# brown-ivl/manus

Measured on AMD Instinct MI355X. Metric: train iters/sec (fwd+bwd) 300k Gaussians @1080p, 8 views; PSNR parity, higher is better.
Workload: dtype f32

## Files before the change

### manus_amd/csrc/image_loss.hip

```cpp
#include "mgr_common.h"
#include "il_list.h"
#include <cstdlib>

#define IL_ACC_SLOTS 64
#define IL_NX (IL_ND + 2 * IL_H1)

struct IlWindow {
    float g[11];
};

typedef mgr_v2f v2f;
__device__ __forceinline__ v2f il_v2(float a) { v2f r = {a, a}; return r; }

__global__ __launch_bounds__(IL_T) void k_image_loss(int H, int W, const float* __restrict__ pred,
                                                     const float* __restrict__ target, IlWindow win, float w_l1,
                                                     float w_ssim, float grad_scale, float* __restrict__ dL_dpred,
                                                     float2* __restrict__ partial, const uint32_t* __restrict__ work_list,
                                                     const uint32_t* __restrict__ work_count, int gxb, int gyb,
                                                     unsigned long long* __restrict__ acc_slots, uint32_t nb, float sum_lim,
                                                     uint32_t* __restrict__ bad_flag) {
    __shared__ v2f s_mix[5][3][IL_NX];
    __shared__ float s_red[4];
    const int tid = threadIdx.x;
    const uint32_t n_work = min(*work_count, nb);
    long long acc_l1 = 0, acc_ss = 0;
    unsigned long long acc_px = 0;
    bool bad = false;
  for (uint32_t wi = blockIdx.x; wi < n_work; wi += gridDim.x) {
    const uint32_t bid = work_list[wi];
    const int bxi = (int)(bid % (uint32_t)gxb), byi = (int)((bid / (uint32_t)gxb) % (uint32_t)gyb), v = (int)(bid / (uint32_t)(gxb * gyb));
    const int w0 = bxi * IL_W, h0 = byi * 2;
    const bool row1 = h0 + 1 < H;
    __syncthreads();
    const size_t plane = (size_t)H * W;
    const float* px = pred + (size_t)v * 3 * plane + (size_t)h0 * W;
    const float* py = target + (size_t)v * 3 * plane + (size_t)h0 * W;
    const v2f m0 = il_v2(win.g[5]), m1 = il_v2(win.g[4]), m2 = il_v2(win.g[3]);

    for (int t = tid; t < IL_NX; t += IL_T) {
        const int w = w0 - 2 * IL_H1 + t;
        v2f x[3], y[3];
#pragma unroll
        for (int c = 0; c < 3; ++c) x[c] = y[c] = il_v2(0.f);
        if (w >= 0 && w < W) {
#pragma unroll
            for (int c = 0; c < 3; ++c) {
                x[c].x = px[c * plane + w];
                y[c].x = py[c * plane + w];
                if (row1) {
                    x[c].y = px[c * plane + W + w];
                    y[c].y = py[c * plane + W + w];
                }
            }
        }
        const v2f q[5][3] = {{x[0], x[1], x[2]},
                             {y[0], y[1], y[2]},
                             {x[0] * x[0], x[1] * x[1], x[2] * x[2]},
                             {y[0] * y[0], y[1] * y[1], y[2] * y[2]},
                             {x[0] * y[0], x[1] * y[1], x[2] * y[2]}};
#pragma unroll
        for (int s5 = 0; s5 < 5; ++s5) {
            s_mix[s5][0][t] = m0 * q[s5][0] + m1 * q[s5][1] + m2 * q[s5][2];
            s_mix[s5][1][t] = m1 * q[s5][0] + m0 * q[s5][1] + m1 * q[s5][2];
            s_mix[s5][2][t] = m2 * q[s5][0] + m1 * q[s5][1] + m0 * q[s5][2];
        }
    }
    __syncthreads();

    const float C1 = 0.01f * 0.01f, C2 = 0.03f * 0.03f;
    const int u0 = 2 * tid;
    v2f ssim_acc = il_v2(0.f);
    v2f d[2][3][3];
#pragma unroll
    for (int c = 0; c < 3; ++c) {
        v2f e[2][5];
#pragma unroll
        for (int s5 = 0; s5 < 5; ++s5) {
            v2f win12[12];
#pragma unroll
            for (int k = 0; k < 12; ++k) win12[k] = s_mix[s5][c][u0 + k];
            v2f a = il_v2(0.f), b = il_v2(0.f);
#pragma unroll
            for (int i = 0; i < 11; ++i) {
                const v2f gi = il_v2(win.g[i]);
                a += gi * win12[i];
                b += gi * win12[i + 1];
            }
            e[0][s5] = a;
            e[1][s5] = b;
        }
#pragma unroll
        for (int pp = 0; pp < 2; ++pp) {
            const int w = w0 - IL_H1 + u0 + pp;
            const v2f mu1 = e[pp][0], mu2 = e[pp][1];
            const v2f s11 = e[pp][2] - mu1 * mu1, s22 = e[pp][3] - mu2 * mu2, s12 = e[pp][4] - mu1 * mu2;
            const v2f A = 2.f * mu1 * mu2 + C1, B = 2.f * s12 + C2;
            const v2f Cc = mu1 * mu1 + mu2 * mu2 + C1, Dd = s11 + s22 + C2;
            v2f iC, iD;
            iC.x = __builtin_amdgcn_rcpf(Cc.x); iC.y = __builtin_amdgcn_rcpf(Cc.y);
            iD.x = __builtin_amdgcn_rcpf(Dd.x); iD.y = __builtin_amdgcn_rcpf(Dd.y);
            const v2f inv = iC * iD;
            const v2f S = A * B * inv;
            const bool okw = w >= 0 && w < W;
            v2f keep = {okw ? 1.f : 0.f, (okw && row1) ? 1.f : 0.f};
            const bool own = u0 + pp >= IL_H1 && u0 + pp < IL_H1 + IL_W;
            if (own) ssim_acc += S * keep;
            d[pp][0][c] = keep * (2.f * mu2 * (B - A) * inv - S * 2.f * mu1 * iC + S * 2.f * mu1 * iD);
            d[pp][1][c] = keep * (-S * iD);
            d[pp][2][c] = keep * (2.f * A * inv);
        }
    }
    __syncthreads();
#pragma unroll
    for (int pp = 0; pp < 2; ++pp) {
#pragma unroll
        for (int k = 0; k < 3; ++k) {
            const v2f a = d[pp][k][0], b = d[pp][k][1], c = d[pp][k][2];
            s_mix[k][0][u0 + pp] = m0 * a + m1 * b + m2 * c;
            s_mix[k][1][u0 + pp] = m1 * a + m0 * b + m1 * c;
            s_mix[k][2][u0 + pp] = m2 * a + m1 * b + m0 * c;
        }
    }
    __syncthreads();

    v2f l1_acc = il_v2(0.f);
    const int o0 = 2 * tid;
    if (o0 < IL_W) {
#pragma unroll
        for (int c = 0; c < 3; ++c) {
            v2f f[2][3];
#pragma unroll
            for (int k = 0; k < 3; ++k) {
                v2f win12[12];
#pragma unroll
                for (int j = 0; j < 12; ++j) win12[j] = s_mix[k][c][o0 + j];
                v2f a = il_v2(0.f), b = il_v2(0.f);
#pragma unroll
                for (int i = 0; i < 11; ++i) {
                    const v2f gi = il_v2(win.g[i]);
                    a += gi * win12[i];
                    b += gi * win12[i + 1];
                }
                f[0][k] = a;
                f[1][k] = b;
            }
#pragma unroll
            for (int pp = 0; pp < 2; ++pp) {
                const int w = w0 + o0 + pp;
                if (o0 + pp < IL_W && w < W) {
                    v2f x, y;
                    x.x = px[c * plane + w];
                    y.x = py[c * plane + w];
                    x.y = row1 ? px[c * plane + W + w] : 0.f;
                    y.y = row1 ? py[c * plane + W + w] : 0.f;
                    const v2f dS = f[pp][0] + 2.f * x * f[pp][1] + y * f[pp][2];
                    const v2f df = x - y;
                    v2f ad = {fabsf(df.x), fabsf(df.y)};
                    l1_acc += ad;
                    const v2f sgn = {df.x > 0.f ? 1.f : (df.x < 0.f ? -1.f : 0.f), df.y > 0.f ? 1.f : (df.y < 0.f ? -1.f : 0.f)};
                    const v2f gr = grad_scale * (w_l1 * sgn - w_ssim * dS);
                    float* go = dL_dpred + (size_t)v * 3 * plane + (size_t)h0 * W + c * plane + w;
                    go[0] = gr.x;
                    if (row1) go[W] = gr.y;
                }
            }
        }
    }
    float l1_sum = mgr_wave_sum63(l1_acc.x + l1_acc.y);
    float ssim_sum = mgr_wave_sum63(ssim_acc.x + ssim_acc.y);
    if ((tid & 63) == 63) {
        s_red[tid >> 6] = l1_sum;
        s_red[2 + (tid >> 6)] = ssim_sum;
    }
    __syncthreads();
    if (tid == 0) {
        const float pa = s_red[0] + s_red[1], pb = s_red[2] + s_red[3];
        partial[bid] = make_float2(pa, pb);
        bad |= !(fabsf(pa) <= sum_lim && fabsf(pb) <= sum_lim);
        acc_l1 += __double2ll_rn((double)pa * 4294967296.0);
        acc_ss += __double2ll_rn((double)pb * 4294967296.0);
        acc_px += (unsigned long long)((min((bxi + 1) * IL_W, W) - bxi * IL_W) * 3 * (row1 ? 2 : 1));
    }
  }
    if (tid == 0 && acc_px) {
        unsigned long long* sl = acc_slots + 3 * (blockIdx.x & (IL_ACC_SLOTS - 1));
        atomicAdd(sl, (unsigned long long)acc_l1);
        atomicAdd(sl + 1, (unsigned long long)acc_ss);
        atomicAdd(sl + 2, acc_px);
        if (bad) atomicOr(bad_flag, 1u);
    }
}

__global__ __launch_bounds__(ILS_T) void k_image_loss_scan(int H, int W, int gxb, const float* __restrict__ pred,
                                                           const float* __restrict__ target, float* __restrict__ dL_dpred,
                                                           float2* __restrict__ partial, uint32_t* __restrict__ work_list,
                                                           uint32_t* __restrict__ work_count) {
    __shared__ uint32_t s_diff[ILS_MAXW / 32];
    __shared__ uint32_t s_ident[(ILS_MAXW / IL_W + 32) / 32];
    const int tid = threadIdx.x;
    const int h0 = blockIdx.x * 2, v = blockIdx.y;
    const bool row1 = h0 + 1 < H;
    const size_t plane = (size_t)H * W;
    const float* px = pred + (size_t)v * 3 * plane + (size_t)h0 * W;
    const float* py = target + (size_t)v * 3 * plane + (size_t)h0 * W;
    float* pg = dL_dpred + (size_t)v * 3 * plane + (size_t)h0 * W;
    const int nwords = (W + 31) / 32;
    for (int k = tid; k < nwords; k += ILS_T) s_diff[k] = 0;
    if (tid < (int)(sizeof(s_ident) / 4)) s_ident[tid] = 0;
    __syncthreads();
    const int rows = row1 ? 2 : 1;
    const bool vec = (W & 3) == 0 && ((((uintptr_t)pred) | ((uintptr_t)target) | ((uintptr_t)dL_dpred)) & 15) == 0;
    if (vec) {
        const int n4 = W >> 2;
        for (int q = tid; q < n4; q += ILS_T) {
            uint32_t d = 0;
#pragma unroll
            for (int c = 0; c < 3; ++c)
                for (int r = 0; r < rows; ++r) {
                    const float4 a = *(const float4*)(px + c * plane + (size_t)r * W + 4 * q);
                    const float4 b = *(const float4*)(py + c * plane + (size_t)r * W + 4 * q);
                    d |= (a.x != b.x ? 1u : 0u) | (a.y != b.y ? 2u : 0u) | (a.z != b.z ? 4u : 0u) | (a.w != b.w ? 8u : 0u);
                }
            if (d) atomicOr(&s_diff[q >> 3], d << ((q & 7) * 4));
        }
    } else {
        for (int w = tid; w < W; w += ILS_T) {
            uint32_t d = 0;
#pragma unroll
            for (int c = 0; c < 3; ++c)
                for (int r = 0; r < rows; ++r) d |= px[c * plane + (size_t)r * W + w] != py[c * plane + (size_t)r * W + w] ? 1u : 0u;
            if (d) atomicOr(&s_diff[w >> 5], 1u << (w & 31));
        }
    }
    __syncthreads();
    for (int b = tid; b < gxb; b += ILS_T) {
        const int lo = max(b * IL_W - 2 * IL_H1, 0), hi = min(b * IL_W + IL_ND, W);
        uint32_t any = 0;
        for (int k = lo >> 5; k <= (hi - 1) >> 5; ++k) {
            uint32_t m = s_diff[k];
            const int base = k << 5;
            if (lo > base) m &= ~0u << (lo - base);
            if (hi < base + 32) m &= ~0u >> (base + 32 - hi);
            any |= m;
        }
        const uint32_t bid = ((uint32_t)v * gridDim.x + blockIdx.x) * (uint32_t)gxb + (uint32_t)b;
        if (any) {
            work_list[atomicAdd(work_count, 1u)] = bid;
        } else {
            atomicOr(&s_ident[b >> 5], 1u << (b & 31));
            const int wcnt = min((b + 1) * IL_W, W) - b * IL_W;
            partial[bid] = make_float2(0.f, (float)(wcnt * 3 * rows));
        }
    }
    __syncthreads();
    if (vec) {
        const int n4 = W >> 2;
        for (int q = tid; q < n4; q += ILS_T) {
            const int w = 4 * q, b0 = w / IL_W, b1 = (w + 3) / IL_W;
            const bool i0 = (s_ident[b0 >> 5] >> (b0 & 31)) & 1u, i1 = (s_ident[b1 >> 5] >> (b1 & 31)) & 1u;
            if (i0 && i1) {
#pragma unroll
                for (int c = 0; c < 3; ++c)
                    for (int r = 0; r < rows; ++r) *(float4*)(pg + c * plane + (size_t)r * W + w) = make_float4(0.f, 0.f, 0.f, 0.f);
            } else if (i0 || i1) {
                for (int e = 0; e < 4; ++e) {
                    const int be = (w + e) / IL_W;
                    if ((s_ident[be >> 5] >> (be & 31)) & 1u)
                        for (int c = 0; c < 3; ++c)
                            for (int r = 0; r < rows; ++r) pg[c * plane + (size_t)r * W + w + e] = 0.f;
                }
            }
        }
    } else {
        for (int w = tid; w < W; w += ILS_T) {
            const int b = w / IL_W;
            if ((s_ident[b >> 5] >> (b & 31)) & 1u)
                for (int c = 0; c < 3; ++c)
                    for (int r = 0; r < rows; ++r) pg[c * plane + (size_t)r * W + w] = 0.f;
        }
    }
}

__global__ __launch_bounds__(ILS_T) void k_image_loss_list(int H, int W, int gxb, const float* __restrict__ target,
                                                           const float* __restrict__ bg, const uint32_t* __restrict__ tile_start,
                                                           float2* __restrict__ partial, uint32_t* __restrict__ work_list,
                                                           uint32_t* __restrict__ work_count, const uint32_t* __restrict__ tmap,
                                                           uint32_t* __restrict__ tmap_out) {
    __shared__ uint32_t s_diff[ILS_MAXW / 32];
    __shared__ uint32_t s_cand[(ILS_MAXW / IL_W + 32) / 32];
    __shared__ uint32_t s_n, s_base;
    const int tid = threadIdx.x;
    if (tid == 0) s_n = 0;
    const int h0 = blockIdx.x * 2, v = blockIdx.y;
    const bool row1 = h0 + 1 < H;
    const size_t plane = (size_t)H * W;
    const float* py = target + (size_t)v * 3 * plane + (size_t)h0 * W;
    const int nwords = (W + 31) / 32;
    const int gxt = (W + 15) / 16, T = gxt * ((H + 15) / 16);
    const uint32_t* trow = tile_start + (size_t)v * T + (size_t)(h0 >> 4) * gxt;
    const size_t map_row = ((size_t)v * gridDim.x + blockIdx.x) * (size_t)nwords;
    for (int k = tid; k < nwords; k += ILS_T) s_diff[k] = tmap ? tmap[map_row + k] : 0u;
    if (tid < (int)(sizeof(s_cand) / 4)) s_cand[tid] = 0;
    __syncthreads();
    if (tile_start)
    for (int b = tid; b < gxb; b += ILS_T) {
        const int lo = max(b * IL_W - 2 * IL_H1, 0), hi = min(b * IL_W + IL_ND, W);
        const int t0 = lo >> 4, t1 = (hi - 1) >> 4;
        if (trow[t1 + 1] == trow[t0]) atomicOr(&s_cand[b >> 5], 1u << (b & 31));
    }
    const int rows = row1 ? 2 : 1;
    const float b0 = bg[0], b1 = bg[1], b2 = bg[2];
    const bool vec = (W & 3) == 0 && (((uintptr_t)target) & 15) == 0;
    if (tmap) {
    } else if (vec) {
        const int n4 = W >> 2;
        for (int q = tid; q < n4; q += ILS_T) {
            uint32_t d = 0;
            for (int rr = 0; rr < rows; ++rr) {
                const float4 c0 = *(const float4*)(py + (size_t)rr * W + 4 * q), c1 = *(const float4*)(py + plane + (size_t)rr * W + 4 * q),
                             c2 = *(const float4*)(py + 2 * plane + (size_t)rr * W + 4 * q);
                d |= ((c0.x != b0 || c1.x != b1 || c2.x != b2) ? 1u : 0u) | ((c0.y != b0 || c1.y != b1 || c2.y != b2) ? 2u : 0u) |
                     ((c0.z != b0 || c1.z != b1 || c2.z != b2) ? 4u : 0u) | ((c0.w != b0 || c1.w != b1 || c2.w != b2) ? 8u : 0u);
            }
            if (d) atomicOr(&s_diff[q >> 3], d << ((q & 7) * 4));
        }
    } else {
        for (int w = tid; w < W; w += ILS_T) {
            uint32_t d = 0;
            for (int rr = 0; rr < rows; ++rr)
                d |= (py[(size_t)rr * W + w] != b0 || py[plane + (size_t)rr * W + w] != b1 || py[2 * plane + (size_t)rr * W + w] != b2) ? 1u : 0u;
            if (d) atomicOr(&s_diff[w >> 5], 1u << (w & 31));
        }
    }
    __syncthreads();
    if (tmap_out) {
        for (int k = tid; k < nwords; k += ILS_T) tmap_out[map_row + k] = s_diff[k];
        if (!tile_start) return;
    }
    uint32_t my_rank[(ILS_MAXW / IL_W + ILS_T) / ILS_T];
    int nmine = 0;
    for (int b = tid; b < gxb; b += ILS_T, ++nmine) {
        const int lo = max(b * IL_W - 2 * IL_H1, 0), hi = min(b * IL_W + IL_ND, W);
        uint32_t any = ((s_cand[b >> 5] >> (b & 31)) & 1u) ? 0u : 1u;
        for (int k = lo >> 5; k <= (hi - 1) >> 5 && !any; ++k) {
            uint32_t m = s_diff[k];
            const int base = k << 5;
            if (lo > base) m &= ~0u << (lo - base);
            if (hi < base + 32) m &= ~0u >> (base + 32 - hi);
            any |= m;
        }
        my_rank[nmine] = any ? atomicAdd(&s_n, 1u) : 0xFFFFFFFFu;
        if (!any) {
            const uint32_t bid = ((uint32_t)v * gridDim.x + blockIdx.x) * (uint32_t)gxb + (uint32_t)b;
            const int wcnt = min((b + 1) * IL_W, W) - b * IL_W;
            partial[bid] = make_float2(0.f, (float)(wcnt * 3 * rows));
        }
    }
    __syncthreads();
    if (tid == 0 && s_n) s_base = atomicAdd(work_count, s_n);
    __syncthreads();
    nmine = 0;
    for (int b = tid; b < gxb; b += ILS_T, ++nmine)
        if (my_rank[nmine] != 0xFFFFFFFFu)
            work_list[s_base + my_rank[nmine]] = ((uint32_t)v * gridDim.x + blockIdx.x) * (uint32_t)gxb + (uint32_t)b;
}

__global__ __launch_bounds__(ILS_T) void k_image_loss_list_mapped(IlListArgs a) {
    __shared__ uint32_t s2[2];
    il_list_mapped_block(a, (int)blockIdx.x, (int)blockIdx.y, s2);
}

__global__ __launch_bounds__(IL_ACC_SLOTS) void k_image_loss_fold(unsigned long long* __restrict__ acc_slots, long long total_px3,
                                                                  float* __restrict__ sums, float ca, float cb, float cc,
                                                                  uint32_t* __restrict__ work_count) {
    __shared__ unsigned long long s_fin[3 * IL_ACC_SLOTS];
    const int tid = threadIdx.x;
#pragma unroll
    for (int q = 0; q < 3; ++q) {
        s_fin[q * IL_ACC_SLOTS + tid] = acc_slots[3 * tid + q];
        acc_slots[3 * tid + q] = 0ull;
    }
    __syncthreads();
    if (tid == 0) {
        long long t_l1 = 0, t_ss = 0;
        unsigned long long t_px = 0;
        for (int k = 0; k < IL_ACC_SLOTS; ++k) {
            t_l1 += (long long)s_fin[k];
            t_ss += (long long)s_fin[IL_ACC_SLOTS + k];
            t_px += s_fin[2 * IL_ACC_SLOTS + k];
        }
        const double ta = (double)t_l1 * (1.0 / 4294967296.0);
        const double tb = (double)t_ss * (1.0 / 4294967296.0) + (double)((unsigned long long)total_px3 - t_px);
        const bool bad = work_count[1] != 0u;
        const float qnan = __int_as_float(0x7FC00000);
        sums[0] = bad ? qnan : (float)ta;
        sums[1] = bad ? qnan : (float)tb;
        sums[2] = bad ? qnan : (float)((double)ca * ta + (double)cb * tb + (double)cc);
        work_count[0] = 0u;
        work_count[1] = 0u;
    }
}


static size_t il_slots_offset(int64_t nb) { return (((size_t)nb * (sizeof(float2) + sizeof(uint32_t)) + 256) + 63) & ~(size_t)63; }
extern "C" size_t mgr_image_loss_workspace_bytes(int V, int H, int W) {
    if (V <= 0 || H <= 0 || W <= 0) return 0;
    return il_slots_offset(il_blocks(V, H, W)) + 3 * IL_ACC_SLOTS * sizeof(unsigned long long);
}

static int image_loss_impl(int V, int H, int W, const float* pred, const float* target, const float* bg3,
                           const uint32_t* tile_start, float w_l1, float w_ssim, float grad_scale, float loss_offset,
                           float* dL_dpred, float* sums, void* workspace, size_t workspace_bytes, void* stream_, int phase = 0,
                           const uint32_t* tmap = nullptr, bool clean = false) {
    if (V <= 0 || H <= 0 || W <= 0) return mgr_fail(MGR_EINVAL, "mgr_image_loss: bad sizes");
    if ((!target && !(phase == 1 && tmap)) || !workspace || (phase != 1 && (!pred || !dL_dpred || !sums))) return mgr_fail(MGR_EINVAL, "mgr_image_loss: null pointer");
    if (H > 65535 || V > 65535) return mgr_fail(MGR_EINVAL, "mgr_image_loss: H and V must fit a grid dimension");
    if (workspace_bytes < mgr_image_loss_workspace_bytes(V, H, W))
        return mgr_fail(MGR_ENOMEM, "mgr_image_loss: workspace too small");
    hipStream_t stream = (hipStream_t)stream_;
    IlWindow win;
    float sum = 0.f;
    for (int i = 0; i < 11; ++i) {
        win.g[i] = (float)exp(-(double)((i - 5) * (i - 5)) / (2.0 * 1.5 * 1.5));
        sum += win.g[i];
    }
    for (int i = 0; i < 11; ++i) win.g[i] /= sum;
    const dim3 grid((W + IL_W - 1) / IL_W, (H + 1) / 2, V);
    const int64_t nb = il_blocks(V, H, W);
    if (nb >= (1ll << 32)) return mgr_fail(MGR_EINVAL, "mgr_image_loss: image batch too large");
    float2* partial = (float2*)workspace;
    uint32_t* work_list = (uint32_t*)((char*)workspace + (size_t)nb * sizeof(float2));
    uint32_t* work_count = (uint32_t*)((char*)workspace + (size_t)nb * (sizeof(float2) + sizeof(uint32_t)) + 64);
    if (W > ILS_MAXW) return mgr_fail(MGR_EINVAL, "mgr_image_loss: image wider than 16384");
    unsigned long long* acc_slots = (unsigned long long*)((char*)workspace + il_slots_offset(nb));
    if (phase != 2 && !clean)
        MGR_HIP(hipMemsetAsync(work_count, 0, (size_t)((char*)(acc_slots + 3 * IL_ACC_SLOTS) - (char*)work_count), stream));
    if (phase == 2) {
    } else if (tile_start && tmap) {
        MGR_PROF("k_image_loss_list", stream);
        const IlListArgs la = il_list_args(V, H, W, tmap, tile_start, workspace);
        hipLaunchKernelGGL(k_image_loss_list_mapped, dim3((unsigned)la.nbx, V), dim3(ILS_T), 0, stream, la);
    } else if (tile_start) {
        MGR_PROF("k_image_loss_list", stream);
        hipLaunchKernelGGL(k_image_loss_list, dim3(grid.y, V), dim3(ILS_T), 0, stream, H, W, (int)grid.x, target, bg3, tile_start,
                           partial, work_list, work_count, tmap, (uint32_t*)nullptr);
    } else {
        MGR_PROF("k_image_loss_scan", stream);
        hipLaunchKernelGGL(k_image_loss_scan, dim3(grid.y, V), dim3(ILS_T), 0, stream, H, W, (int)grid.x, pred, target, dL_dpred,
                           partial, work_list, work_count);
    }
    if (phase == 1) return MGR_OK;
    {
        MGR_PROF("k_image_loss", stream);
#ifndef IL_GRID
#define IL_GRID (256 * 5)
#endif
        const int64_t pb = nb < IL_GRID ? nb : IL_GRID;
        const float sum_lim = (float)(2147483648.0 * (1.0 - 1.0 / 1048576.0) / (double)nb);
        hipLaunchKernelGGL(k_image_loss, dim3((unsigned)pb), dim3(IL_T), 0, stream, H, W, pred, target, win, w_l1, w_ssim,
                           grad_scale, dL_dpred, partial, (const uint32_t*)work_list, (const uint32_t*)work_count,
                           (int)grid.x, (int)grid.y, acc_slots, (uint32_t)nb, sum_lim, work_count + 1);
    }
    hipLaunchKernelGGL(k_image_loss_fold, dim3(1), dim3(IL_ACC_SLOTS), 0, stream, acc_slots, (long long)V * H * W * 3,
                       sums, grad_scale * w_l1, -grad_scale * w_ssim, loss_offset, work_count);
    MGR_LAUNCH_CHECK("k_image_loss", stream, 0);
    return MGR_OK;
}

extern "C" int mgr_image_loss(int V, int H, int W, const float* pred, const float* target, float w_l1, float w_ssim,
                              float grad_scale, float loss_offset, float* dL_dpred, float* sums, void* workspace,
                              size_t workspace_bytes, void* stream_) {
    return image_loss_impl(V, H, W, pred, target, nullptr, nullptr, w_l1, w_ssim, grad_scale, loss_offset, dL_dpred, sums,
                           workspace, workspace_bytes, stream_);
}

extern "C" int mgr_image_loss_tiles(int V, int H, int W, const float* pred, const float* target, const float* bg3,
                                    const uint32_t* tile_start, float w_l1, float w_ssim, float grad_scale, float loss_offset,
                                    float* dL_dpred, float* sums, void* workspace, size_t workspace_bytes, void* stream_) {
    if (!bg3 || !tile_start) return mgr_fail(MGR_EINVAL, "mgr_image_loss_tiles: null pointer");
    return image_loss_impl(V, H, W, pred, target, bg3, tile_start, w_l1, w_ssim, grad_scale, loss_offset, dL_dpred, sums,
                           workspace, workspace_bytes, stream_);
}

extern "C" int mgr_image_loss_tiles_list(int V, int H, int W, const float* target, const float* bg3, const uint32_t* tile_start,
                                         void* workspace, size_t workspace_bytes, void* stream_) {
    if (!bg3 || !tile_start) return mgr_fail(MGR_EINVAL, "mgr_image_loss_tiles_list: null pointer");
    return image_loss_impl(V, H, W, nullptr, target, bg3, tile_start, 0.f, 0.f, 0.f, 0.f, nullptr, nullptr, workspace,
                           workspace_bytes, stream_, 1);
}

extern "C" int mgr_image_loss_tiles_finish(int V, int H, int W, const float* pred, const float* target, float w_l1, float w_ssim,
                                           float grad_scale, float loss_offset, float* dL_dpred, float* sums, void* workspace,
                                           size_t workspace_bytes, void* stream_) {
    return image_loss_impl(V, H, W, pred, target, nullptr, nullptr, w_l1, w_ssim, grad_scale, loss_offset, dL_dpred, sums,
                           workspace, workspace_bytes, stream_, 2);
}

extern "C" size_t mgr_image_loss_target_map_words(int V, int H, int W) {
    if (V <= 0 || H <= 0 || W <= 0) return 0;
    return (size_t)V * ((H + 1) / 2) * ((W + 31) / 32);
}

extern "C" int mgr_image_loss_target_map(int V, int H, int W, const float* target, const float* bg3, uint32_t* map, void* stream_) {
    if (V <= 0 || H <= 0 || W <= 0) return mgr_fail(MGR_EINVAL, "mgr_image_loss_target_map: bad sizes");
    if (!target || !bg3 || !map) return mgr_fail(MGR_EINVAL, "mgr_image_loss_target_map: null pointer");
    if (H > 65535 || V > 65535 || W > ILS_MAXW) return mgr_fail(MGR_EINVAL, "mgr_image_loss_target_map: image too large");
    hipLaunchKernelGGL(k_image_loss_list, dim3((H + 1) / 2, V), dim3(ILS_T), 0, (hipStream_t)stream_, H, W, (W + IL_W - 1) / IL_W,
                       target, bg3, (const uint32_t*)nullptr, (float2*)nullptr, (uint32_t*)nullptr, (uint32_t*)nullptr,
                       (const uint32_t*)nullptr, map);
    MGR_LAUNCH_CHECK("k_image_loss_list", (hipStream_t)stream_, 0);
    return MGR_OK;
}

extern "C" int mgr_image_loss_tiles_list_mapped(int V, int H, int W, const uint32_t* map, const float* bg3, const uint32_t* tile_start,
                                                void* workspace, size_t workspace_bytes, int workspace_kept, void* stream_) {
    if (!map || !bg3 || !tile_start) return mgr_fail(MGR_EINVAL, "mgr_image_loss_tiles_list_mapped: null pointer");
    return image_loss_impl(V, H, W, nullptr, nullptr, bg3, tile_start, 0.f, 0.f, 0.f, 0.f, nullptr, nullptr, workspace,
                           workspace_bytes, stream_, 1, map, workspace_kept != 0);
}
```

Baseline: 775.0.

## Restructure SSIM loss kernel with register-held tiles and software-prefetched next work item

Rewrites the fused L1+SSIM loss kernel so each thread keeps its own pixel pair in registers, prefetches the next work item's pixels while the current one is still being processed, and recomputes the per-channel vertical mix into a smaller shared buffer instead of one large 5x3 shared array. Pixels reused in the gradient stage come from registers rather than being reloaded from global memory. Loads and gradient stores are vectorised as float2 when alignment allows. It also pins waves-per-EU and raises the grid size. The extra barriers per channel and the higher register pressure could offset the gains.

Result: no change. 775.3 (median of 2 runs) (+0.0%).

```diff
diff --git a/manus_amd/csrc/image_loss.hip b/manus_amd/csrc/image_loss.hip
--- a/manus_amd/csrc/image_loss.hip
+++ b/manus_amd/csrc/image_loss.hip
@@ -12,73 +12,157 @@
 typedef mgr_v2f v2f;
 __device__ __forceinline__ v2f il_v2(float a) { v2f r = {a, a}; return r; }
 
-__global__ __launch_bounds__(IL_T) void k_image_loss(int H, int W, const float* __restrict__ pred,
-                                                     const float* __restrict__ target, IlWindow win, float w_l1,
-                                                     float w_ssim, float grad_scale, float* __restrict__ dL_dpred,
-                                                     float2* __restrict__ partial, const uint32_t* __restrict__ work_list,
-                                                     const uint32_t* __restrict__ work_count, int gxb, int gyb,
-                                                     unsigned long long* __restrict__ acc_slots, uint32_t nb, float sum_lim,
-                                                     uint32_t* __restrict__ bad_flag) {
-    __shared__ v2f s_mix[5][3][IL_NX];
+typedef float il_v4f __attribute__((ext_vector_type(4)));
+
+struct IlSpan {
+    int bxi, w0, h0, v;
+    bool row1;
+    size_t base;
+};
+__device__ __forceinline__ IlSpan il_span(uint32_t bid, int gxb, int gyb, int H, int W, size_t plane) {
+    IlSpan s;
+    s.bxi = (int)(bid % (uint32_t)gxb);
+    const int byi = (int)((bid / (uint32_t)gxb) % (uint32_t)gyb);
+    s.v = (int)(bid / (uint32_t)(gxb * gyb));
+    s.w0 = s.bxi * IL_W;
+    s.h0 = byi * 2;
+    s.row1 = s.h0 + 1 < H;
+    s.base = (size_t)s.v * 3 * plane + (size_t)s.h0 * W;
+    return s;
+}
+
+__device__ __forceinline__ void il_load_pair(const float* __restrict__ px, const float* __restrict__ py, size_t plane, int W, int w,
+                                             bool row1, bool vec2, v2f (&x)[2][3], v2f (&y)[2][3]) {
+    const bool in0 = w >= 0 && w < W, in1 = w + 1 >= 0 && w + 1 < W;
+    const int r1 = row1 ? W : 0;
+    if (vec2) {
+        const uint32_t wc = in0 ? (uint32_t)w : 0u;
+#pragma unroll
+        for (int c = 0; c < 3; ++c) {
+            const float* pxc = px + c * plane;
+            const float* pyc = py + c * plane;
+            const float2 a0 = *(const float2*)(pxc + wc), a1 = *(const float2*)(pxc + r1 + wc);
+            const float2 b0 = *(const float2*)(pyc + wc), b1 = *(const float2*)(pyc + r1 + wc);
+            x[0][c].x = in0 ? a0.x : 0.f; x[0][c].y = (in0 && row1) ? a1.x : 0.f;
+            x[1][c].x = in0 ? a0.y : 0.f; x[1][c].y = (in0 && row1) ? a1.y : 0.f;
+            y[0][c].x = in0 ? b0.x : 0.f; y[0][c].y = (in0 && row1) ? b1.x : 0.f;
+            y[1][c].x = in0 ? b0.y : 0.f; y[1][c].y = (in0 && row1) ? b1.y : 0.f;
+        }
+    } else {
+        const uint32_t wc0 = in0 ? (uint32_t)w : 0u, wc1 = in1 ? (uint32_t)(w + 1) : 0u;
+#pragma unroll
+        for (int c = 0; c < 3; ++c) {
+            const float* pxc = px + c * plane;
+            const float* pyc = py + c * plane;
+            const float a00 = pxc[wc0], a01 = (pxc + r1)[wc0], a10 = pxc[wc1], a11 = (pxc + r1)[wc1];
+            const float b00 = pyc[wc0], b01 = (pyc + r1)[wc0], b10 = pyc[wc1], b11 = (pyc + r1)[wc1];
+            x[0][c].x = in0 ? a00 : 0.f; x[0][c].y = (in0 && row1) ? a01 : 0.f;
+            x[1][c].x = in1 ? a10 : 0.f; x[1][c].y = (in1 && row1) ? a11 : 0.f;
+            y[0][c].x = in0 ? b00 : 0.f; y[0][c].y = (in0 && row1) ? b01 : 0.f;
+            y[1][c].x = in1 ? b10 : 0.f; y[1][c].y = (in1 && row1) ? b11 : 0.f;
+        }
+    }
+}
+
+__device__ __forceinline__ void il_mix5(const v2f (&x)[3], const v2f (&y)[3], int c, v2f m0, v2f m1, v2f m2, v2f (&o)[5]) {
+    const v2f q[5][3] = {{x[0], x[1], x[2]},
+                         {y[0], y[1], y[2]},
+                         {x[0] * x[0], x[1] * x[1], x[2] * x[2]},
+                         {y[0] * y[0], y[1] * y[1], y[2] * y[2]},
+                         {x[0] * y[0], x[1] * y[1], x[2] * y[2]}};
+#pragma unroll
+    for (int s5 = 0; s5 < 5; ++s5) {
+        if (c == 0) o[s5] = m0 * q[s5][0] + m1 * q[s5][1] + m2 * q[s5][2];
+        else if (c == 1) o[s5] = m1 * q[s5][0] + m0 * q[s5][1] + m1 * q[s5][2];
+        else o[s5] = m2 * q[s5][0] + m1 * q[s5][1] + m0 * q[s5][2];
+    }
+}
+
+__global__ __launch_bounds__(IL_T) __attribute__((amdgpu_waves_per_eu(4, 4))) void k_image_loss(
+    int H, int W, const float* __restrict__ pred, const float* __restrict__ target, IlWindow win, float w_l1, float w_ssim,
+    float grad_scale, float* __restrict__ dL_dpred, float2* __restrict__ partial, const uint32_t* __restrict__ work_list,
+    const uint32_t* __restrict__ work_count, int gxb, int gyb, unsigned long long* __restrict__ acc_slots, uint32_t nb, float sum_lim,
+    uint32_t* __restrict__ bad_flag) {
+    __shared__ __attribute__((aligned(16))) v2f s_rows[9][IL_NX];
+    __shared__ __attribute__((aligned(16))) v2f s_left[6][2 * IL_H1];
     __shared__ float s_red[4];
     const int tid = threadIdx.x;
     const uint32_t n_work = min(*work_count, nb);
+    if (blockIdx.x >= n_work) return;
     long long acc_l1 = 0, acc_ss = 0;
     unsigned long long acc_px = 0;
     bool bad = false;
-  for (uint32_t wi = blockIdx.x; wi < n_work; wi += gridDim.x) {
+    const size_t plane = (size_t)H * W;
+    const bool vec2 = (W & 1) == 0 && ((((uintptr_t)pred) | ((uintptr_t)target)) & 7) == 0;
+    const bool vec2s = (W & 1) == 0 && (((uintptr_t)dL_dpred) & 7) == 0;
+    const v2f m0 = il_v2(win.g[5]), m1 = il_v2(win.g[4]), m2 = il_v2(win.g[3]);
+    const float C1 = 0.01f * 0.01f, C2 = 0.03f * 0.03f;
+    const int u0 = 2 * tid, o0 = 2 * tid;
+    const int te = 2 * min(tid, IL_H1 - 1);
+
+    uint32_t wi = blockIdx.x;
+    IlSpan sp = il_span(work_list[wi], gxb, gyb, H, W, plane);
+    v2f x[2][3], y[2][3];
+    v2f xe[2][3], ye[2][3];
+    il_load_pair(pred + sp.base, target + sp.base, plane, W, sp.w0 + 2 * tid, sp.row1, vec2, x, y);
+    il_load_pair(pred + sp.base, target + sp.base, plane, W, sp.w0 - 2 * IL_H1 + te, sp.row1, vec2, xe, ye);
+  for (;;) {
     const uint32_t bid = work_list[wi];
-    const int bxi = (int)(bid % (uint32_t)gxb), byi = (int)((bid / (uint32_t)gxb) % (uint32_t)gyb), v = (int)(bid / (uint32_t)(gxb * gyb));
-    const int w0 = bxi * IL_W, h0 = byi * 2;
-    const bool row1 = h0 + 1 < H;
-    __syncthreads();
-    const size_t plane = (size_t)H * W;
-    const float* px = pred + (size_t)v * 3 * plane + (size_t)h0 * W;
-    const float* py = target + (size_t)v * 3 * plane + (size_t)h0 * W;
-    const v2f m0 = il_v2(win.g[5]), m1 = il_v2(win.g[4]), m2 = il_v2(win.g[3]);
-
-    for (int t = tid; t < IL_NX; t += IL_T) {
-        const int w = w0 - 2 * IL_H1 + t;
-        v2f x[3], y[3];
-#pragma unroll
-        for (int c = 0; c < 3; ++c) x[c] = y[c] = il_v2(0.f);
-        if (w >= 0 && w < W) {
-#pragma unroll
-            for (int c = 0; c < 3; ++c) {
-                x[c].x = px[c * plane + w];
-                y[c].x = py[c * plane + w];
-                if (row1) {
-                    x[c].y = px[c * plane + W + w];
-                    y[c].y = py[c * plane + W + w];
-                }
-            }
-        }
-        const v2f q[5][3] = {{x[0], x[1], x[2]},
-                             {y[0], y[1], y[2]},
-                             {x[0] * x[0], x[1] * x[1], x[2] * x[2]},
-                             {y[0] * y[0], y[1] * y[1], y[2] * y[2]},
-                             {x[0] * y[0], x[1] * y[1], x[2] * y[2]}};
-#pragma unroll
-        for (int s5 = 0; s5 < 5; ++s5) {
-            s_mix[s5][0][t] = m0 * q[s5][0] + m1 * q[s5][1] + m2 * q[s5][2];
-            s_mix[s5][1][t] = m1 * q[s5][0] + m0 * q[s5][1] + m1 * q[s5][2];
-            s_mix[s5][2][t] = m2 * q[s5][0] + m1 * q[s5][1] + m0 * q[s5][2];
-        }
-    }
-    __syncthreads();
-
-    const float C1 = 0.01f * 0.01f, C2 = 0.03f * 0.03f;
-    const int u0 = 2 * tid;
+    const uint32_t wn = wi + gridDim.x;
+    const bool more = wn < n_work;
+    const IlSpan ns = il_span(work_list[more ? wn : wi], gxb, gyb, H, W, plane);
+    const int w0 = sp.w0;
+    const bool row1 = sp.row1;
+    if (tid < IL_H1) {
+#pragma unroll
+        for (int cc = 0; cc < 3; ++cc) {
+            const il_v4f px2 = {xe[0][cc].x, xe[0][cc].y, xe[1][cc].x, xe[1][cc].y}, py2 = {ye[0][cc].x, ye[0][cc].y, ye[1][cc].x, ye[1][cc].y};
+            *(il_v4f*)&s_left[cc][2 * tid] = px2;
+            *(il_v4f*)&s_left[3 + cc][2 * tid] = py2;
+        }
+    }
+
     v2f ssim_acc = il_v2(0.f);
     v2f d[2][3][3];
 #pragma unroll
     for (int c = 0; c < 3; ++c) {
+        {
+#pragma unroll
+            for (int pp = 0; pp < 2; ++pp)
+#pragma unroll
+                for (int cc = 0; cc < 3; ++cc) asm("" : "+v"(x[pp][cc]), "+v"(y[pp][cc]));
+            v2f ma[5], mb[5];
+            il_mix5(x[0], y[0], c, m0, m1, m2, ma);
+            il_mix5(x[1], y[1], c, m0, m1, m2, mb);
+#pragma unroll
+            for (int s5 = 0; s5 < 5; ++s5) {
+                const il_v4f pr = {ma[s5].x, ma[s5].y, mb[s5].x, mb[s5].y};
+                *(il_v4f*)&s_rows[s5][2 * IL_H1 + 2 * tid] = pr;
+            }
+            if (tid < IL_H1) {
+                v2f lx[2][3], ly[2][3];
+#pragma unroll
+                for (int cc = 0; cc < 3; ++cc) {
+                    const il_v4f px2 = *(const il_v4f*)&s_left[cc][2 * tid], py2 = *(const il_v4f*)&s_left[3 + cc][2 * tid];
+                    lx[0][cc] = {px2.x, px2.y}; lx[1][cc] = {px2.z, px2.w};
+                    ly[0][cc] = {py2.x, py2.y}; ly[1][cc] = {py2.z, py2.w};
+                }
+                il_mix5(lx[0], ly[0], c, m0, m1, m2, ma);
+                il_mix5(lx[1], ly[1], c, m0, m1, m2, mb);
+#pragma unroll
+                for (int s5 = 0; s5 < 5; ++s5) {
+                    const il_v4f pr = {ma[s5].x, ma[s5].y, mb[s5].x, mb[s5].y};
+                    *(il_v4f*)&s_rows[s5][2 * tid] = pr;
+                }
+            }
+        }
+        __syncthreads();
         v2f e[2][5];
 #pragma unroll
         for (int s5 = 0; s5 < 5; ++s5) {
             v2f win12[12];
 #pragma unroll
-            for (int k = 0; k < 12; ++k) win12[k] = s_mix[s5][c][u0 + k];
+            for (int k = 0; k < 12; ++k) win12[k] = s_rows[s5][u0 + k];
             v2f a = il_v2(0.f), b = il_v2(0.f);
 #pragma unroll
             for (int i = 0; i < 11; ++i) {
@@ -86,6 +170,7 @@
                 a += gi * win12[i];
                 b += gi * win12[i + 1];
             }
+            asm volatile("" : "+v"(a), "+v"(b) : : "memory");
             e[0][s5] = a;
             e[1][s5] = b;
         }
@@ -109,23 +194,52 @@
             d[pp][1][c] = keep * (-S * iD);
             d[pp][2][c] = keep * (2.f * A * inv);
         }
-    }
-    __syncthreads();
-#pragma unroll
-    for (int pp = 0; pp < 2; ++pp) {
-#pragma unroll
-        for (int k = 0; k < 3; ++k) {
+        asm volatile("" : "+v"(ssim_acc));
+        if (c == 0) {
+#pragma unroll
+            for (int k = 0; k < 3; ++k) {
+                const il_v4f pk = {d[0][k][0].x, d[0][k][0].y, d[1][k][0].x, d[1][k][0].y};
+                *(il_v4f*)&s_rows[5 + k][u0] = pk;
+            }
+        } else if (c == 1) {
+            const il_v4f pk = {d[0][0][1].x, d[0][0][1].y, d[1][0][1].x, d[1][0][1].y};
+            *(il_v4f*)&s_rows[8][u0] = pk;
+        }
+        __syncthreads();
+    }
+#pragma unroll
+    for (int k = 0; k < 3; ++k) {
+        const il_v4f pk = *(const il_v4f*)&s_rows[5 + k][u0];
+        d[0][k][0] = {pk.x, pk.y}; d[1][k][0] = {pk.z, pk.w};
+    }
+    {
+        const il_v4f pk = *(const il_v4f*)&s_rows[8][u0];
+        d[0][0][1] = {pk.x, pk.y}; d[1][0][1] = {pk.z, pk.w};
+    }
+#pragma unroll
+    for (int k = 0; k < 3; ++k) {
+        v2f r[2][3];
+#pragma unroll
+        for (int pp = 0; pp < 2; ++pp) {
             const v2f a = d[pp][k][0], b = d[pp][k][1], c = d[pp][k][2];
-            s_mix[k][0][u0 + pp] = m0 * a + m1 * b + m2 * c;
-            s_mix[k][1][u0 + pp] = m1 * a + m0 * b + m1 * c;
-            s_mix[k][2][u0 + pp] = m2 * a + m1 * b + m0 * c;
-        }
-    }
+            r[pp][0] = m0 * a + m1 * b + m2 * c;
+            r[pp][1] = m1 * a + m0 * b + m1 * c;
+            r[pp][2] = m2 * a + m1 * b + m0 * c;
+        }
+#pragma unroll
+        for (int c = 0; c < 3; ++c) {
+            const il_v4f pr = {r[0][c].x, r[0][c].y, r[1][c].x, r[1][c].y};
+            *(il_v4f*)&s_rows[3 * k + c][u0] = pr;
+        }
+    }
+    v2f nx[2][3], ny[2][3], nxe[2][3], nye[2][3];
+    il_load_pair(pred + ns.base, target + ns.base, plane, W, ns.w0 + 2 * tid, ns.row1, vec2, nx, ny);
+    il_load_pair(pred + ns.base, target + ns.base, plane, W, ns.w0 - 2 * IL_H1 + te, ns.row1, vec2, nxe, nye);
     __syncthreads();
 
     v2f l1_acc = il_v2(0.f);
-    const int o0 = 2 * tid;
     if (o0 < IL_W) {
+        float* gbase = dL_dpred + sp.base;
 #pragma unroll
         for (int c = 0; c < 3; ++c) {
             v2f f[2][3];
@@ -133,7 +247,7 @@
             for (int k = 0; k < 3; ++k) {
                 v2f win12[12];
 #pragma unroll
-                for (int j = 0; j < 12; ++j) win12[j] = s_mix[k][c][o0 + j];
+                for (int j = 0; j < 12; ++j) win12[j] = s_rows[3 * k + c][o0 + j];
                 v2f a = il_v2(0.f), b = il_v2(0.f);
 #pragma unroll
                 for (int i = 0; i < 11; ++i) {
@@ -141,28 +255,35 @@
                     a += gi * win12[i];
                     b += gi * win12[i + 1];
                 }
+                asm volatile("" : "+v"(a), "+v"(b) : : "memory");
                 f[0][k] = a;
                 f[1][k] = b;
             }
+            v2f gr2[2];
 #pragma unroll
             for (int pp = 0; pp < 2; ++pp) {
                 const int w = w0 + o0 + pp;
+                gr2[pp] = il_v2(0.f);
                 if (o0 + pp < IL_W && w < W) {
-                    v2f x, y;
-                    x.x = px[c * plane + w];
-                    y.x = py[c * plane + w];
-                    x.y = row1 ? px[c * plane + W + w] : 0.f;
-                    y.y = row1 ? py[c * plane + W + w] : 0.f;
-                    const v2f dS = f[pp][0] + 2.f * x * f[pp][1] + y * f[pp][2];
-                    const v2f df = x - y;
+                    const v2f xo = x[pp][c], yo = y[pp][c];
+                    const v2f dS = f[pp][0] + 2.f * xo * f[pp][1] + yo * f[pp][2];
+                    const v2f df = xo - yo;
                     v2f ad = {fabsf(df.x), fabsf(df.y)};
                     l1_acc += ad;
                     const v2f sgn = {df.x > 0.f ? 1.f : (df.x < 0.f ? -1.f : 0.f), df.y > 0.f ? 1.f : (df.y < 0.f ? -1.f : 0.f)};
                     const v2f gr = grad_scale * (w_l1 * sgn - w_ssim * dS);
-                    float* go = dL_dpred + (size_t)v * 3 * plane + (size_t)h0 * W + c * plane + w;
-                    go[0] = gr.x;
-                    if (row1) go[W] = gr.y;
+                    gr2[pp] = gr;
+                    if (!vec2s) {
+                        float* go = gbase + c * plane + w;
+                        go[0] = gr.x;
+                        if (row1) go[W] = gr.y;
+                    }
                 }
+            }
+            if (vec2s && w0 + o0 < W) {
+                float* go = gbase + c * plane + w0 + o0;
+                *(float2*)go = make_float2(gr2[0].x, gr2[1].x);
+                if (row1) *(float2*)(go + W) = make_float2(gr2[0].y, gr2[1].y);
             }
         }
     }
@@ -179,8 +300,18 @@
         bad |= !(fabsf(pa) <= sum_lim && fabsf(pb) <= sum_lim);
         acc_l1 += __double2ll_rn((double)pa * 4294967296.0);
         acc_ss += __double2ll_rn((double)pb * 4294967296.0);
-        acc_px += (unsigned long long)((min((bxi + 1) * IL_W, W) - bxi * IL_W) * 3 * (row1 ? 2 : 1));
-    }
+        acc_px += (unsigned long long)((min((sp.bxi + 1) * IL_W, W) - sp.bxi * IL_W) * 3 * (row1 ? 2 : 1));
+    }
+    if (!more) break;
+    wi = wn;
+    sp = ns;
+#pragma unroll
+    for (int pp = 0; pp < 2; ++pp)
+#pragma unroll
+        for (int c = 0; c < 3; ++c) {
+            x[pp][c] = nx[pp][c]; y[pp][c] = ny[pp][c];
+            xe[pp][c] = nxe[pp][c]; ye[pp][c] = nye[pp][c];
+        }
   }
     if (tid == 0 && acc_px) {
         unsigned long long* sl = acc_slots + 3 * (blockIdx.x & (IL_ACC_SLOTS - 1));
@@ -453,7 +584,7 @@
     {
         MGR_PROF("k_image_loss", stream);
 #ifndef IL_GRID
-#define IL_GRID (256 * 5)
+#define IL_GRID (256 * 8)
 #endif
         const int64_t pb = nb < IL_GRID ? nb : IL_GRID;
         const float sum_lim = (float)(2147483648.0 * (1.0 - 1.0 / 1048576.0) / (double)nb);
```
